# HowToSD/cremage

Measured on AMD Instinct MI355X. Metric: images/sec SD1.5 512x512 20-step Euler ancestral (txt2img, CFG 7.5, incl. VAE decode), higher is better.
Workload: dtype bf16; 1 GPU; SD1.5 txt2img 512x512, batch 4 per GPU, 20-step Euler ancestral, bf16 UNet (B=8 with CFG) + fp32-class (split-bf16 x3) VAE decode, synthetic name-keyed weights, synthetic conditioning; sampler=euler_a, sampler_steps=20, parallelism=batch-sharded x1 (weights broadcast 0.00 GB once, images all-gathered per step)

## Files before the change

### cremage_amd/csrc/attention.hip

```cpp
#include "crg_common.h"
#include <stdlib.h>
#include <type_traits>

namespace {

struct AttnP {
  const bf16* q; const bf16* k; const bf16* vt; bf16* o;
  long ldq, ldk, ldvt, ldo;
  int B, H, Nq, Nk, Dh;
  float scale_log2;
};

#ifdef CRG_ATTN_LAPS
__device__ unsigned long long crg_attn_laps[32 * 8];
#define LAP(i)                                       \
  do {                                               \
    const unsigned long long now_ = wall_clock64(); \
    lap[i] += now_ - tl;                             \
    tl = now_;                                       \
  } while (0)
#else
#define LAP(i)
#endif

// ... 835 lines not shown
  constexpr int Dh = KC * 8;
#ifdef CRG_ATTN_NO_QPAD
  constexpr bool QPAD = false;
#else
  constexpr bool QPAD = (KC & 1) && ONES;
#endif
  constexpr float QPAD_T = 10.0f;
  __shared__ __attribute__((aligned(256))) char smem[2 * KBYTES + 2 * VBYTES];

  const int t = threadIdx.x;
  const int lane = t & 63;
  const int wave = __builtin_amdgcn_readfirstlane(t >> 6);
  const int r = lane & 31, hh = lane >> 5;
  int bx = blockIdx.x, by = blockIdx.y;
  {
    const int nqb = gridDim.x, total = nqb * gridDim.y;
    if ((total & 7) == 0) {
      const int id = bx + nqb * by;
      const int L = (id & 7) * (total >> 3) + (id >> 3);
      by = L / nqb;
      bx = L - by * nqb;
    }
  }
  const int b = by / p.H, h = by % p.H;
  const int q0 = bx * (32 * NW) + wave * 32;
  const bf16* Q = p.q + (long)b * p.Nq * p.ldq + (long)h * Dh;
  const bf16* K = p.k + (long)b * p.Nk * p.ldk + (long)h * Dh;
  const bf16* VT = p.vt + ((long)b * p.H + h) * Dh * p.ldvt;
  bf16* O = p.o + (long)b * p.Nq * p.ldo + (long)h * Dh;

  int voff[NQ];
#pragma unroll
  for (int q = 0; q < NQ; ++q) {
    const int j = wave + NW * q;
    if (j < KC) {
      const int i = 64 * j + lane;
      const int rho = i / KC, cpos = i - rho * KC;
      const int c = cpos ^ AttnKSwz<KC>::of(rho);
      const int key = (rho & ~12) | ((rho & 4) << 1) | ((rho & 8) >> 1);
      voff[q] = (int)(key * p.ldk * 2) + c * 16;
    } else {
      const int i = 64 * (j - KC) + lane;
      const int d = i >> 3, cpos = i & 7;
      const int c = cpos ^ ((d >> 1) & 7);
      voff[q] = (int)(d * p.ldvt * 2) + c * 16;
    }
  }
  const int T = p.Nk >> 6;
  auto issue = [&](int kt, int vt) {
#pragma unroll
    for (int q = 0; q < NQ; ++q) {
      const int j = wave + NW * q;
      if (j < KC) {
        if (kt >= 0) attn_dma16(K, k_bytes, smem + (kt & 1) * KBYTES + j * 1024, voff[q], kt * 64 * (int)p.ldk * 2);
      } else if (j < NI) {
        if (vt >= 0) attn_dma16(VT, v_bytes, smem + 2 * KBYTES + (vt & 1) * VBYTES + (j - KC) * 1024, voff[q], vt * 128);
      }
    }
  };

  if (t < 32) {
    const int st = t >> 4, row = (t >> 3) & 1, ch = t & 7;
    const bf16 one = (bf16)1.0f;
    const bf16x8 ones8 = {one, one, one, one, one, one, one, one};
    const bf16x8 zero8 = {0, 0, 0, 0, 0, 0, 0, 0};
    *reinterpret_cast<bf16x8*>(smem + 2 * KBYTES + st * VBYTES + (Dh + row) * 128 + ch * 16) = (ONES && row == 0) ? ones8 : zero8;
  }

  bf16x8 qf[KS];
  {
    const bf16x8 zero8 = {0, 0, 0, 0, 0, 0, 0, 0};
    const int query = q0 + r;
#pragma unroll
    for (int s = 0; s < KS; ++s) {
      const int d0 = 16 * s + 8 * hh;
      qf[s] = (query < p.Nq && d0 < Dh) ? *reinterpret_cast<const bf16x8*>(Q + (long)query * p.ldq + d0) : zero8;
      if (QPAD) {
#pragma unroll
        for (int j = 0; j < 8; ++j) qf[s][j] = (bf16)((float)qf[s][j] * p.scale_log2);
      }
    }
  }
  float m_ref = 0.f;
  f32x16 oacc[NV];
#pragma unroll
  for (int i = 0; i < NV; ++i)
#pragma unroll
    for (int e = 0; e < 16; ++e) oacc[i][e] = 0.f;
  float m_run = -INFINITY, l_run = 0.f;
  f32x16 st[2][2];
  bf16x8 pf[2][2][2];

  const int kaddr = r * (KC * 16) + ((hh ^ AttnKSwz<KC>::of(r)) << 4);
  const int kaddr_last = (KC & 1) ? r * (KC * 16) : kaddr;
  const int ones_addr = 2 * KBYTES + Dh * 128;
  int vaddr[NV];
#pragma unroll
  for (int dv = 0; dv < NV; ++dv) {
    const int R = dv * 32 + r;
    const int lrow = R < Dh + 1 ? R : Dh + 1;
    vaddr[dv] = 2 * KBYTES + lrow * 128 + ((((lrow >> 1) & 7) ^ hh) << 4);
  }

  auto qk = [&](int kt, f32x16 (&dst)[2]) {
    const char* Ks = smem + (kt & 1) * KBYTES;
#pragma unroll
    for (int kb = 0; kb < 2; ++kb) {
#pragma unroll
      for (int e = 0; e < 16; ++e) dst[kb][e] = 0.f;
#pragma unroll
      for (int s = 0; s < KS; ++s) {
        const int base = ((KC & 1) && s == KS - 1) ? kaddr_last : kaddr;
        const int lo = ((2 * s) & (SPAN - 1)) << 4, hi = ((2 * s) & ~(SPAN - 1)) << 4;
        const char* ka = Ks + ((base ^ lo) + hi + kb * 32 * KC * 16);
        if (QPAD && s == KS - 1) ka = hh ? smem + ones_addr : ka;
        const bf16x8 kf = *reinterpret_cast<const bf16x8*>(ka);
        dst[kb] = CRG_MFMA_32x32x16(kf, qf[s], dst[kb]);
      }
    }
  };
  auto pv = [&](int vt, const bf16x8 (&pp)[2][2]) {
    const char* Vs = smem + (vt & 1) * VBYTES;
#pragma unroll
    for (int dv = 0; dv < NV; ++dv) {
      const int va = vaddr[dv];
#pragma unroll
      for (int kb = 0; kb < 2; ++kb)
#pragma unroll
        for (int s2 = 0; s2 < 2; ++s2) {
          const bf16x8 vf = *reinterpret_cast<const bf16x8*>(Vs + (va ^ ((kb * 4 + 2 * s2) << 4)));
          oacc[dv] = CRG_MFMA_32x32x16(vf, pp[kb][s2], oacc[dv]);
        }
    }
  };
  auto tile_end = [&]() {
    attn_wait_vm0();
    __syncthreads();
  };
  auto step = [&](int tt, auto c_c, auto pv_c, auto qk_c) {
    constexpr int C = decltype(c_c)::value;
    constexpr bool PV = decltype(pv_c)::value, QK = decltype(qk_c)::value;
    constexpr int NPV = PV ? 4 * NV : 0, NQK = QK ? 2 * KS : 0, G = NPV + NQK;
    constexpr int ITEMS = 21;
    __builtin_amdgcn_sched_barrier(0);
    issue(tt + 2, tt);
#ifndef CRG_ATTN_SP_DEPTH
#define CRG_ATTN_SP_DEPTH 2
#endif
    constexpr int D = CRG_ATTN_SP_DEPTH;
    bf16x8 fr[G];
    const char* Vs = smem + ((tt - 1) & 1) * VBYTES;
    const char* Ks = smem + ((tt + 1) & 1) * KBYTES;
    auto fetch = [&](int g) {
      if (PV && g < NPV) {
        fr[g] = *reinterpret_cast<const bf16x8*>(Vs + (vaddr[g >> 2] ^ ((((g >> 1) & 1) * 4 + 2 * (g & 1)) << 4)));
      } else {
        const int i = g - NPV, kb = i / KS, s = i - kb * KS;
        const int base = ((KC & 1) && s == KS - 1) ? kaddr_last : kaddr;
        const int lo = ((2 * s) & (SPAN - 1)) << 4, hi = ((2 * s) & ~(SPAN - 1)) << 4;
        const char* ka = Ks + ((base ^ lo) + hi + kb * 32 * KC * 16);
        if (QPAD && s == KS - 1) ka = hh ? smem + ones_addr : ka;
        fr[g] = *reinterpret_cast<const bf16x8*>(ka);
      }
    };
#pragma unroll
    for (int g = 0; g < (D < G ? D : G); ++g) fetch(g);
    __builtin_amdgcn_sched_barrier(0);
    float mx = -INFINITY, m_new = 0.f, alpha = 1.f, rs = 0.f;
    f32x16(&sc)[2] = st[C];
    auto item = [&](int it) {
      if (it < 4) {
        const int kb = it >> 1, e0 = 8 * (it & 1);
        mx = fmaxf(fmaxf(mx, sc[kb][e0]), sc[kb][e0 + 1]);
        mx = fmaxf(fmaxf(mx, sc[kb][e0 + 2]), sc[kb][e0 + 3]);
        mx = fmaxf(fmaxf(mx, sc[kb][e0 + 4]), sc[kb][e0 + 5]);
        mx = fmaxf(fmaxf(mx, sc[kb][e0 + 6]), sc[kb][e0 + 7]);
      } else if (it == 4) {
        if constexpr (QPAD) {
          mx = attn_max_halves(mx);
          const bool move = !PV || mx > QPAD_T;
          if (__any(move)) {
            const float want = m_ref + mx;
            const bf16 r_hi = (bf16)want;
            const bf16 r_lo = (bf16)(want - (float)r_hi);
            const float ref_new = move ? (float)r_hi + (float)r_lo : m_ref;
            const float delta = ref_new - m_ref;
            m_ref = ref_new;
            alpha = __builtin_amdgcn_exp2f(-delta);
#pragma unroll
            for (int kb = 0; kb < 2; ++kb)
#pragma unroll
              for (int e = 0; e < 16; ++e) sc[kb][e] -= delta;
            if (move && hh) {
              qf[KS - 1][0] = (bf16)(-(float)r_hi);
              qf[KS - 1][1] = (bf16)(-(float)r_lo);
            }
          }
        } else {
          mx = attn_max_halves(mx) * p.scale_log2;
          m_new = fmaxf(m_run, mx);
          alpha = __builtin_amdgcn_exp2f(m_run - m_new);
          m_run = m_new;
        }
      } else {
        const int j = it - 5, kb = j >> 3, e = 2 * (j & 7);
        float x0, x1;
        if constexpr (QPAD) {
          x0 = sc[kb][e];
          x1 = sc[kb][e + 1];
        } else {
          x0 = __builtin_fmaf(sc[kb][e], p.scale_log2, -m_new);
          x1 = __builtin_fmaf(sc[kb][e + 1], p.scale_log2, -m_new);
        }
        const float p0 = __builtin_amdgcn_exp2f(x0), p1 = __builtin_amdgcn_exp2f(x1);
        if (!ONES) rs += p0 + p1;
        pf[C][kb][e >> 3][e & 7] = (bf16)p0;
        pf[C][kb][e >> 3][(e & 7) + 1] = (bf16)p1;
      }
    };
#pragma unroll
    for (int g = 0; g < G; ++g) {
      if (g + D < G) fetch(g + D);
      if (PV && g < NPV) {
        oacc[g >> 2] = CRG_MFMA_32x32x16(fr[g], pf[1 - C][(g >> 1) & 1][g & 1], oacc[g >> 2]);
      } else {
        const int i = g - NPV, kb = i / KS, s = i - kb * KS;
        if (s == 0) {
#pragma unroll
          for (int e = 0; e < 16; ++e) st[1 - C][kb][e] = 0.f;
        }
        st[1 - C][kb] = CRG_MFMA_32x32x16(fr[g], qf[s], st[1 - C][kb]);
      }
#pragma unroll
      for (int it = g * ITEMS / G; it < (g + 1) * ITEMS / G; ++it) item(it);
      __builtin_amdgcn_sched_barrier(0);
    }
    if (!ONES) l_run = l_run * alpha + rs;
#if defined(__HIP_DEVICE_COMPILE__)
    asm volatile("" : "+v"(pf[C][0][0]), "+v"(pf[C][0][1]), "+v"(pf[C][1][0]), "+v"(pf[C][1][1]));
#endif
    if (__any(alpha != 1.0f)) {
#pragma unroll
      for (int i = 0; i < NV; ++i)
#pragma unroll
        for (int e = 0; e < 16; ++e) oacc[i][e] *= alpha;
    }
    tile_end();
  };
  using I0 = std::integral_constant<int, 0>;
  using I1 = std::integral_constant<int, 1>;
  using TT = std::true_type;
  using FF = std::false_type;

  issue(0, -1);
  issue(1, -1);
  tile_end();
  qk(0, st[0]);
  __syncthreads();
  step(0, I0{}, FF{}, TT{});
  for (int tt = 1; tt + 1 < T; tt += 2) {
    step(tt, I1{}, TT{}, TT{});
    step(tt + 1, I0{}, TT{}, TT{});
  }
  step(T - 1, I1{}, TT{}, FF{});
  pv(T - 1, pf[1]);

  float l_tot;
  if (ONES) {
    constexpr int dvl = Dh >> 5, regl = ((Dh & 31) >> 3) * 4;
    const float v = oacc[dvl < NV ? dvl : 0][regl];
    const float other = __shfl_xor(v, 32);
    l_tot = hh == 0 ? v : other;
  } else {
    l_tot = l_run + __shfl_xor(l_run, 32);
  }
  const float inv = 1.0f / l_tot;
  const int query = q0 + r;
  if (query < p.Nq) {
#pragma unroll
    for (int dv = 0; dv < NV; ++dv)
#pragma unroll
      for (int g = 0; g < 4; ++g) {
        const int d = dv * 32 + 8 * g + 4 * hh;
        if (d < Dh) {
          bf16x4 o4;
#pragma unroll
          for (int e = 0; e < 4; ++e) o4[e] = (bf16)(oacc[dv][4 * g + e] * inv);
          *reinterpret_cast<bf16x4*>(O + (long)query * p.ldo + d) = o4;
        }
      }
  }
}

template <int KC, int NV, int NW, int OCC>
int launch_attn_sp(crg_ctx* ctx, hipStream_t st, const AttnP& p) {
  dim3 grid((p.Nq + 32 * NW - 1) / (32 * NW), p.B * p.H);
  const unsigned k_bytes = (unsigned)((((long)p.Nk - 1) * p.ldk + p.Dh) * 2);
  const unsigned v_bytes = (unsigned)((((long)p.Dh - 1) * p.ldvt + (p.Nk + 7) / 8 * 8) * 2);
  hipLaunchKernelGGL((attn_sp_kernel<KC, NV, (KC * 8 < NV * 32), NW, OCC>), grid, dim3(64 * NW), 0, st, p, k_bytes, v_bytes);
  CRG_CHECK_LAUNCH(ctx, "attention (software-pipelined)");
  return 0;
}

template <int KS, int NV>
int launch_attn_ctx(crg_ctx* ctx, hipStream_t st, const AttnP& p, bool vrm) {
  const int nqg = (p.Nq + 127) / 128, bh = p.B * p.H;
  int gx = 1;
  for (int d = 1; d <= nqg; ++d)
    if (nqg % d == 0 && (long)d * bh <= 1024) gx = d;
  dim3 grid(gx, bh);
  if (vrm) {
    if (p.Dh < NV * 32) hipLaunchKernelGGL((attn_ctx_kernel<KS, NV, true, true>), grid, dim3(256), 0, st, p);
    else hipLaunchKernelGGL((attn_ctx_kernel<KS, NV, false, true>), grid, dim3(256), 0, st, p);
  } else {
    if (p.Dh < NV * 32) hipLaunchKernelGGL((attn_ctx_kernel<KS, NV, true, false>), grid, dim3(256), 0, st, p);
    else hipLaunchKernelGGL((attn_ctx_kernel<KS, NV, false, false>), grid, dim3(256), 0, st, p);
  }
  CRG_CHECK_LAUNCH(ctx, "attention (few keys)");
  return 0;
}

template <int KS, int NV>
int launch_attn(crg_ctx* ctx, hipStream_t st, const AttnP& p, bool vrm) {
  dim3 grid((p.Nq + 127) / 128, p.B * p.H);
  if (vrm) {
    if (p.Dh < NV * 32) hipLaunchKernelGGL((attn_kernel<KS, NV, true, true>), grid, dim3(256), 0, st, p);
    else hipLaunchKernelGGL((attn_kernel<KS, NV, false, true>), grid, dim3(256), 0, st, p);
  } else {
    if (p.Dh < NV * 32) hipLaunchKernelGGL((attn_kernel<KS, NV, true>), grid, dim3(256), 0, st, p);
    else hipLaunchKernelGGL((attn_kernel<KS, NV, false>), grid, dim3(256), 0, st, p);
  }
  CRG_CHECK_LAUNCH(ctx, "attention");
  return 0;
}

}

static int attention_entry(crg_ctx* ctx, void* stream, const void* q, int64_t ldq, const void* k, int64_t ldk, const void* v, int64_t ldv,
                           void* o, int64_t ldo, int B, int H, int Nq, int Nk, int Dh, float scale, int dtype, bool vrm) {
  if (!ctx) return -22;
  CRG_REQUIRE(ctx, dtype == CRG_BF16, "attention: only bf16 is implemented (dtype %d)", dtype);
  CRG_REQUIRE(ctx, B > 0 && H > 0 && Nq > 0 && Nk > 0, "attention: empty problem B=%d H=%d Nq=%d Nk=%d", B, H, Nq, Nk);
  CRG_REQUIRE(ctx, Dh % 8 == 0 && Dh >= 8 && Dh <= 160, "attention: head dim %d unsupported (multiple of 8, <= 160)", Dh);
  CRG_REQUIRE(ctx, ldq % 8 == 0 && ldk % 8 == 0 && ldv % 8 == 0 && ldo % 4 == 0, "attention: leading dimensions must keep 16-byte alignment");
  if (vrm) CRG_REQUIRE(ctx, ldv >= (int64_t)H * Dh, "attention: ldv=%ld must cover H*Dh=%d", (long)ldv, H * Dh);
  else CRG_REQUIRE(ctx, ldv >= ((Nk + 7) / 8) * 8, "attention: ldvt=%ld must cover Nk=%d rounded up to 8", (long)ldv, Nk);
  CRG_REQUIRE(ctx, (((uintptr_t)q | (uintptr_t)k | (uintptr_t)v) & 15) == 0 && ((uintptr_t)o & 7) == 0, "attention: pointers must be 16-byte aligned");
  AttnP p{(const bf16*)q, (const bf16*)k, (const bf16*)v, (bf16*)o, (long)ldq, (long)ldk, (long)ldv, (long)ldo, B, H, Nq, Nk, Dh,
          scale * 1.4426950408889634f};
  hipStream_t st = (hipStream_t)stream;
  const double flops = 4.0 * B * H * (double)Nq * Nk * Dh;
  const double bytes = 2.0 * B * H * Dh * (2.0 * Nq + 2.0 * Nk);
  crg_prof_scope ps(ctx, st, CRG_K_ATTN, flops, bytes);
  const int ks = (Dh + 15) / 16;
  static const int use_ctx = getenv("CRG_ATTN_CTX") ? atoi(getenv("CRG_ATTN_CTX")) : 1;
  const int nqg_ = (Nq + 127) / 128;
  if (use_ctx && Nk <= 128 && (long)nqg_ * B * H >= 2048) {
    switch (ks) {
      case 1: return launch_attn_ctx<1, 1>(ctx, st, p, vrm);
      case 2: return launch_attn_ctx<2, 1>(ctx, st, p, vrm);
      case 3: return launch_attn_ctx<3, 2>(ctx, st, p, vrm);
      case 4: return launch_attn_ctx<4, 2>(ctx, st, p, vrm);
      case 5: return launch_attn_ctx<5, 3>(ctx, st, p, vrm);
      case 6: return launch_attn_ctx<6, 3>(ctx, st, p, vrm);
      case 7: return launch_attn_ctx<7, 4>(ctx, st, p, vrm);
      case 8: return launch_attn_ctx<8, 4>(ctx, st, p, vrm);
      case 9: return launch_attn_ctx<9, 5>(ctx, st, p, vrm);
      case 10: return launch_attn_ctx<10, 5>(ctx, st, p, vrm);
    }
  }
  static const int use_dma = getenv("CRG_ATTN_DMA") ? atoi(getenv("CRG_ATTN_DMA")) : 1;
  static const int dma_tail = getenv("CRG_ATTN_TAIL") ? atoi(getenv("CRG_ATTN_TAIL")) : 1;
  if (use_dma && !vrm && (Nk % 64 == 0 || (dma_tail && Nk > 8)) && ((long)Nk * ldk * 2 < (1l << 31)) && ((long)Dh * ldv * 2 < (1l << 31))) {
    const bool sp = use_dma == 1 && Nk % 128 == 0;
    static const int use_occ4 = getenv("CRG_ATTN_OCC4") ? atoi(getenv("CRG_ATTN_OCC4")) : 1;
    if (Dh == 40) {
      if (sp) return use_occ4 ? launch_attn_sp<5, 2, 8, 4>(ctx, st, p) : launch_attn_sp<5, 2, 8, 2>(ctx, st, p);
      return (use_dma == 4 || (use_dma == 1 && Nk <= 256)) ? launch_attn_dma<5, 2, 4, 1, 4>(ctx, st, p) : launch_attn_dma<5, 2, 4, 1, 8>(ctx, st, p);
    }
    if (Dh == 64) {
      if (use_dma == 5 && Nk % 128 == 0) return launch_attn_sp<8, 2, 8, 2>(ctx, st, p);
      return use_dma == 8 ? launch_attn_dma<8, 2, 4, 1, 8>(ctx, st, p) : launch_attn_dma<8, 2, 4, 1, 4>(ctx, st, p);
    }
    if (Dh == 80) {
      if (sp) return launch_attn_sp<10, 3, 8, 2>(ctx, st, p);
      return use_dma == 4 ? launch_attn_dma<10, 3, 3, 1, 4>(ctx, st, p) : launch_attn_dma<10, 3, 2, 1, 8>(ctx, st, p);
    }
  }
  switch (ks) {
    case 1: return launch_attn<1, 1>(ctx, st, p, vrm);
    case 2: return launch_attn<2, 1>(ctx, st, p, vrm);
    case 3: return launch_attn<3, 2>(ctx, st, p, vrm);
    case 4: return launch_attn<4, 2>(ctx, st, p, vrm);
    case 5: return launch_attn<5, 3>(ctx, st, p, vrm);
    case 6: return launch_attn<6, 3>(ctx, st, p, vrm);
    case 7: return launch_attn<7, 4>(ctx, st, p, vrm);
    case 8: return launch_attn<8, 4>(ctx, st, p, vrm);
    case 9: return launch_attn<9, 5>(ctx, st, p, vrm);
    case 10: return launch_attn<10, 5>(ctx, st, p, vrm);
  }
  return crg_fail(ctx, -22, "attention: head dim %d unsupported", Dh);
}

extern "C" int crg_attention(crg_ctx* ctx, void* stream, const void* q, int64_t ldq, const void* k, int64_t ldk,
                             const void* vt, int64_t ldvt, void* o, int64_t ldo, int B, int H, int Nq, int Nk, int Dh,
                             float scale, int dtype) {
  return attention_entry(ctx, stream, q, ldq, k, ldk, vt, ldvt, o, ldo, B, H, Nq, Nk, Dh, scale, dtype, false);
}

extern "C" int crg_attention_v(crg_ctx* ctx, void* stream, const void* q, int64_t ldq, const void* k, int64_t ldk,
                               const void* v, int64_t ldv, void* o, int64_t ldo, int B, int H, int Nq, int Nk, int Dh,
                               float scale, int dtype) {
  return attention_entry(ctx, stream, q, ldq, k, ldk, v, ldv, o, ldo, B, H, Nq, Nk, Dh, scale, dtype, true);
}

#ifdef CRG_ATTN_LAPS
extern "C" int crg_debug_read_attn(unsigned long long* dst, int n) {
  return (int)hipMemcpyFromSymbol(dst, HIP_SYMBOL(crg_attn_laps), sizeof(unsigned long long) * (size_t)n);
}
#endif
```

Baseline: 17.84 images/s.

## Add persistent row-tiled cross-attention kernel keeping K/V resident in LDS

After: 17.79 images/s. About the same (-0.3%).

```diff
diff --git a/cremage_amd/csrc/attention.hip b/cremage_amd/csrc/attention.hip
--- a/cremage_amd/csrc/attention.hip
+++ b/cremage_amd/csrc/attention.hip
@@ -1161,6 +1161,233 @@
   return 0;
 }
 
+constexpr int RW_KEYS = 96, RW_TQ = 32, RW_C = 320, RW_CH = RW_C / 8;
+constexpr int RW_KROW = 656, RW_VROW = 704, RW_QROW = 656;
+constexpr int RW_LDS = RW_KEYS * RW_KROW + RW_KEYS * RW_VROW + RW_TQ * RW_QROW;
+
+template <int DH, int NW>
+__global__ __launch_bounds__(64 * NW, 1) void attn_rows_kernel(AttnP p) {
+  constexpr int KS = (DH + 15) / 16, NV = (KS + 1) / 2, HG = RW_C / DH;
+  constexpr bool ONES = DH < NV * 32;
+  constexpr int NT = 64 * NW;
+  constexpr int QLOADS = (RW_TQ * RW_CH + NT - 1) / NT, KVLOADS = (RW_KEYS * RW_CH + NT - 1) / NT;
+  extern __shared__ __attribute__((aligned(16))) char rsm[];
+  char* const Ks = rsm;
+  char* const Vs = rsm + RW_KEYS * RW_KROW;
+  char* const Qs = Vs + RW_KEYS * RW_VROW;
+
+  const int t = threadIdx.x;
+  const int lane = t & 63;
+  const int wave = __builtin_amdgcn_readfirstlane(t >> 6);
+  const int r = lane & 31, hh = lane >> 5;
+  const int G = p.H * DH / RW_C;
+  const int b = blockIdx.y / G, g = blockIdx.y - b * G;
+  const bf16* Q = p.q + (long)b * p.Nq * p.ldq + g * RW_C;
+  const bf16* K = p.k + (long)b * p.Nk * p.ldk + g * RW_C;
+  const bf16* V = p.vt + (long)b * p.Nk * p.ldvt + g * RW_C;
+  bf16* O = p.o + (long)b * p.Nq * p.ldo + g * RW_C;
+  const bf16x8 zero8 = {0, 0, 0, 0, 0, 0, 0, 0};
+  const int ntq = (p.Nq + RW_TQ - 1) / RW_TQ;
+
+  auto load_q = [&](bf16x8 (&dst)[QLOADS], int qt) {
+#pragma unroll
+    for (int i = 0; i < QLOADS; ++i) {
+      const int idx = t + NT * i, row = idx / RW_CH, c = idx - row * RW_CH;
+      const int query = qt * RW_TQ + row;
+      dst[i] = (idx < RW_TQ * RW_CH && qt < ntq && query < p.Nq) ? *reinterpret_cast<const bf16x8*>(Q + (long)query * p.ldq + c * 8) : zero8;
+    }
+  };
+  bf16x8 qn[QLOADS];
+  load_q(qn, blockIdx.x);
+
+  {
+    bf16x8 kr[KVLOADS], vr[KVLOADS];
+#pragma unroll
+    for (int i = 0; i < KVLOADS; ++i) {
+      const int idx = t + NT * i, key = idx / RW_CH, c = idx - key * RW_CH;
+      const bool ok = idx < RW_KEYS * RW_CH && key < p.Nk;
+      kr[i] = ok ? *reinterpret_cast<const bf16x8*>(K + (long)key * p.ldk + c * 8) : zero8;
+      vr[i] = ok ? *reinterpret_cast<const bf16x8*>(V + (long)key * p.ldvt + c * 8) : zero8;
+    }
+#pragma unroll
+    for (int i = 0; i < KVLOADS; ++i) {
+      const int idx = t + NT * i, key = idx / RW_CH, c = idx - key * RW_CH;
+      if (idx < RW_KEYS * RW_CH) {
+        *reinterpret_cast<bf16x8*>(Ks + key * RW_KROW + c * 16) = kr[i];
+        *reinterpret_cast<bf16x8*>(Vs + key * RW_VROW + c * 16) = vr[i];
+      }
+    }
+    if (t < RW_KEYS) *reinterpret_cast<bf16x8*>(Ks + t * RW_KROW + 2 * RW_C) = zero8;
+    for (int idx = t; idx < RW_KEYS * 4; idx += NT) {
+      bf16x8 v = zero8;
+      if ((idx & 3) == 0) v[0] = (bf16)1.0f;
+      *reinterpret_cast<bf16x8*>(Vs + (idx >> 2) * RW_VROW + 2 * RW_C + (idx & 3) * 16) = v;
+    }
+  }
+
+  const int ktr = (4 * (lane >> 5) + ((lane >> 2) & 3)) * RW_VROW;
+  const int ctr = 16 * ((lane >> 4) & 1) + 4 * (lane & 3);
+
+  for (int qt = blockIdx.x; qt < ntq; qt += gridDim.x) {
+#pragma unroll
+    for (int i = 0; i < QLOADS; ++i) {
+      const int idx = t + NT * i, row = idx / RW_CH, c = idx - row * RW_CH;
+      if (idx < RW_TQ * RW_CH) *reinterpret_cast<bf16x8*>(Qs + row * RW_QROW + c * 16) = qn[i];
+    }
+    __syncthreads();
+    load_q(qn, qt + gridDim.x);
+
+    for (int h = wave; h < HG; h += NW) {
+      const int cb = h * DH;
+      bf16x8 qf[KS];
+      int kofs[KS];
+#pragma unroll
+      for (int s = 0; s < KS; ++s) {
+        const int d0 = 16 * s + 8 * hh;
+        const bool in = (16 * s + 8 < DH) || d0 < DH;
+        qf[s] = in ? *reinterpret_cast<const bf16x8*>(Qs + r * RW_QROW + (cb + d0) * 2) : zero8;
+        kofs[s] = r * RW_KROW + (in ? (cb + d0) * 2 : 2 * RW_C);
+      }
+      int vofs[NV];
+#pragma unroll
+      for (int dv = 0; dv < NV; ++dv) {
+        const int rel = dv * 32 + ctr;
+        vofs[dv] = ktr + ((!ONES || dv * 32 + 32 <= DH || rel < DH) ? cb + rel : RW_C + rel - DH) * 2;
+      }
+      f32x16 oacc[NV];
+#pragma unroll
+      for (int i = 0; i < NV; ++i)
+#pragma unroll
+        for (int e = 0; e < 16; ++e) oacc[i][e] = 0.f;
+      float m_run = -INFINITY, l_run = 0.f;
+
+      auto tile = [&](auto nkb_c, int kbase) {
+        constexpr int NKB = decltype(nkb_c)::value;
+        f32x16 st[NKB];
+#pragma unroll
+        for (int kb = 0; kb < NKB; ++kb) {
+#pragma unroll
+          for (int e = 0; e < 16; ++e) st[kb][e] = 0.f;
+          if (kbase + kb * 32 < p.Nk) {
+#pragma unroll
+            for (int s = 0; s < KS; ++s) {
+              const bf16x8 kf = *reinterpret_cast<const bf16x8*>(Ks + (kbase + kb * 32) * RW_KROW + kofs[s]);
+              st[kb] = CRG_MFMA_32x32x16(kf, qf[s], st[kb]);
+            }
+          }
+        }
+        if (p.Nk < kbase + NKB * 32) {
+#pragma unroll
+          for (int kb = 0; kb < NKB; ++kb)
+#pragma unroll
+            for (int e = 0; e < 16; ++e) {
+              const int key = kbase + kb * 32 + (e & 3) + 8 * (e >> 2) + 4 * hh;
+              if (key >= p.Nk) st[kb][e] = -INFINITY;
+            }
+        }
+        float mx = st[0][0];
+#pragma unroll
+        for (int kb = 0; kb < NKB; ++kb)
+#pragma unroll
+          for (int e = 0; e < 16; ++e) mx = fmaxf(mx, st[kb][e]);
+        mx = fmaxf(mx, __shfl_xor(mx, 32)) * p.scale_log2;
+        const float m_new = fmaxf(m_run, mx);
+        if (__any(m_new != m_run)) {
+          const float alpha = __builtin_amdgcn_exp2f(m_run - m_new);
+          l_run *= alpha;
+#pragma unroll
+          for (int i = 0; i < NV; ++i)
+#pragma unroll
+            for (int e = 0; e < 16; ++e) oacc[i][e] *= alpha;
+          m_run = m_new;
+        }
+        float rs = 0.f;
+#pragma unroll
+        for (int kb = 0; kb < NKB; ++kb) {
+          st[kb] = st[kb] * p.scale_log2 - m_run;
+#pragma unroll
+          for (int e = 0; e < 16; ++e) {
+            const float pe = __builtin_amdgcn_exp2f(st[kb][e]);
+            st[kb][e] = pe;
+            if (!ONES) rs += pe;
+          }
+        }
+        if (!ONES) l_run += rs;
+        bf16x8 pf[NKB][2];
+#pragma unroll
+        for (int kb = 0; kb < NKB; ++kb)
+#pragma unroll
+          for (int s2 = 0; s2 < 2; ++s2)
+#pragma unroll
+            for (int j = 0; j < 8; ++j) pf[kb][s2][j] = (bf16)st[kb][8 * s2 + j];
+        typedef short s16x4 __attribute__((ext_vector_type(4)));
+        typedef __attribute__((address_space(3))) s16x4* trptr_t;
+#pragma unroll
+        for (int dv = 0; dv < NV; ++dv)
+#pragma unroll
+          for (int kb = 0; kb < NKB; ++kb)
+#pragma unroll
+            for (int s2 = 0; s2 < 2; ++s2) {
+              if (kbase + kb * 32 + 16 * s2 >= p.Nk) continue;
+              const char* a0 = Vs + (kbase + kb * 32 + 16 * s2) * RW_VROW + vofs[dv];
+              const s16x4 lo = __builtin_amdgcn_ds_read_tr16_b64_v4i16((trptr_t)a0);
+              const s16x4 hi = __builtin_amdgcn_ds_read_tr16_b64_v4i16((trptr_t)(a0 + 8 * RW_VROW));
+              const short v8[8] = {lo[0], lo[1], lo[2], lo[3], hi[0], hi[1], hi[2], hi[3]};
+              bf16x8 vf;
+              __builtin_memcpy(&vf, v8, 16);
+              oacc[dv] = CRG_MFMA_32x32x16(vf, pf[kb][s2], oacc[dv]);
+            }
+      };
+      tile(std::integral_constant<int, 2>{}, 0);
+      if (p.Nk > 64) tile(std::integral_constant<int, 1>{}, 64);
+
+      float l_tot;
+      if (ONES) {
+        constexpr int dvl = DH >> 5, regl = ((DH & 31) >> 3) * 4;
+        const float v = oacc[dvl < NV ? dvl : 0][regl];
+        const float other = __shfl_xor(v, 32);
+        l_tot = hh == 0 ? v : other;
+      } else {
+        l_tot = l_run + __shfl_xor(l_run, 32);
+      }
+      const float inv = 1.0f / l_tot;
+#pragma unroll
+      for (int dv = 0; dv < NV; ++dv)
+#pragma unroll
+        for (int gq = 0; gq < 4; ++gq) {
+          const int d = dv * 32 + 8 * gq + 4 * hh;
+          if (dv * 32 + 8 * gq + 8 <= DH || d < DH) {
+            bf16x4 o4;
+#pragma unroll
+            for (int e = 0; e < 4; ++e) o4[e] = (bf16)(oacc[dv][4 * gq + e] * inv);
+            *reinterpret_cast<bf16x4*>(Qs + r * RW_QROW + (cb + d) * 2) = o4;
+          }
+        }
+    }
+    __syncthreads();
+#pragma unroll
+    for (int i = 0; i < QLOADS; ++i) {
+      const int idx = t + NT * i, row = idx / RW_CH, c = idx - row * RW_CH;
+      const int query = qt * RW_TQ + row;
+      if (idx < RW_TQ * RW_CH && query < p.Nq) *reinterpret_cast<bf16x8*>(O + (long)query * p.ldo + c * 8) = *reinterpret_cast<const bf16x8*>(Qs + row * RW_QROW + c * 16);
+    }
+  }
+}
+
+template <int DH>
+int launch_attn_rows(crg_ctx* ctx, hipStream_t st, const AttnP& p) {
+  constexpr int NW = RW_C / DH > 4 ? 8 : 4;
+  auto kern = attn_rows_kernel<DH, NW>;
+  if (int rc = crg_set_dyn_lds(ctx, reinterpret_cast<const void*>(kern), RW_LDS, "attention (rows)")) return rc;
+  const int ntq = (p.Nq + RW_TQ - 1) / RW_TQ, bg = p.B * (p.H * DH / RW_C);
+  const int ncu = ctx->n_cu > 0 ? ctx->n_cu : 256;
+  int gx = (ncu + bg - 1) / bg;
+  if (gx > ntq) gx = ntq;
+  hipLaunchKernelGGL(kern, dim3(gx, bg), dim3(64 * NW), RW_LDS, st, p);
+  CRG_CHECK_LAUNCH(ctx, "attention (rows)");
+  return 0;
+}
+
 template <int KS, int NV>
 int launch_attn_ctx(crg_ctx* ctx, hipStream_t st, const AttnP& p, bool vrm) {
   const int nqg = (p.Nq + 127) / 128, bh = p.B * p.H;
@@ -1212,6 +1439,15 @@
   const double bytes = 2.0 * B * H * Dh * (2.0 * Nq + 2.0 * Nk);
   crg_prof_scope ps(ctx, st, CRG_K_ATTN, flops, bytes);
   const int ks = (Dh + 15) / 16;
+  static const int use_rows = getenv("CRG_ATTN_ROWS") ? atoi(getenv("CRG_ATTN_ROWS")) : 1;
+  if (use_rows && vrm && Nk <= RW_KEYS && ((long)H * Dh) % RW_C == 0 && RW_C % Dh == 0 && ldo % 8 == 0 && ((uintptr_t)o & 15) == 0 && (long)B * (H * Dh / RW_C) <= 65535) {
+    const long units = (long)((Nq + RW_TQ - 1) / RW_TQ) * B * (H * Dh / RW_C);
+    const bool all = use_rows == 2;
+    if (Dh == 40) return launch_attn_rows<40>(ctx, st, p);
+    if (Dh == 64 && (all || units <= (ctx->n_cu > 0 ? ctx->n_cu : 256))) return launch_attn_rows<64>(ctx, st, p);
+    if (Dh == 80 && all) return launch_attn_rows<80>(ctx, st, p);
+    if (Dh == 160 && (all || Nk > 64)) return launch_attn_rows<160>(ctx, st, p);
+  }
   static const int use_ctx = getenv("CRG_ATTN_CTX") ? atoi(getenv("CRG_ATTN_CTX")) : 1;
   const int nqg_ = (Nq + 127) / 128;
   if (use_ctx && Nk <= 128 && (long)nqg_ * B * H >= 2048) {
```
